# Gaurav14cs17/Bayer_Low_light_Image_Enhancement

Measured on AMD Instinct MI355X. Metric: megapixels/sec RawFormer-S 512x512 RAW->sRGB, higher is better.
Workload: dtype f32; 1 GPU; RawFormer-S(FLCA) dim=32, batch=8 of packed 4x512x512 synthetic Bayer per GPU; frames_per_gpu=8, variant=flca, weights=synthetic (seeded, random-init scale), parallelism=batch-sharded x1, device=AMD Radeon Graphics

## Files before the change

bayer_low_light_image_enhancement_amd/csrc/rf_gemm1x1.hip:

```cpp
#include <cstdio>
#include <cstdlib>
#include "rf_common.h"

namespace rf {

__device__ __forceinline__ const float* kset_base(const Conv1x1Args& a, int b, int s) {
    const int k = 4 * s;
    const bool first = k < a.C1;
    const float* src = first ? a.x1 : a.x2;
    const size_t off = (size_t)b * (size_t)(first ? a.x1_bstride : a.x2_bstride) + (size_t)(first ? k : k - a.C1) * (size_t)a.P;
    return src + off;
}

__device__ __forceinline__ float4 ldv(const float* __restrict__ base, unsigned off) {
    return *reinterpret_cast<const float4*>(base + off);
}

template <int NCO>
__device__ __forceinline__ void zero_acc(f32x4 (&acc)[NCO][4]) {
#pragma unroll
    for (int t = 0; t < NCO; ++t)
#pragma unroll
        for (int g = 0; g < 4; ++g) acc[t][g] = (f32x4){0.f, 0.f, 0.f, 0.f};
}

template <class BP>
__device__ __forceinline__ void b3_split_pair(float xa, float xb, BP& bp, int g, int hp) {
    unsigned a0, a1, a2, b0, b1, b2;
    b3_split(xa, a0, a1, a2);
    b3_split(xb, b0, b1, b2);
    bp[g][0][hp] = b3_pack(a0, b0);
    bp[g][1][hp] = b3_pack(a1, b1);
    bp[g][2][hp] = b3_pack(a2, b2);
}

template <int NCO, bool RES>
__device__ __forceinline__ void epilogue(const Conv1x1Args& a, f32x4 (&acc)[NCO][4], int tfirst, int ntiles,
                                         const float* __restrict__ bias_l, const float4* res,
                                         int b, int p0, int kq, bool live) {
    const int P = a.P;
    float* outb = a.out + (size_t)b * a.out_bstride;
    if (a.mode == 0) {
        const unsigned voff = (unsigned)(4 * kq) * (unsigned)P + (unsigned)p0;
#pragma unroll
        for (int t = 0; t < NCO; ++t) {
            if (t >= ntiles) break;
#pragma unroll
            for (int r = 0; r < 4; ++r) {
                const int cu = 16 * (tfirst + t) + r;
                const float bs = bias_l[16 * t + 4 * kq + r];
                float v[4] = {acc[t][0][r] + bs, acc[t][1][r] + bs, acc[t][2][r] + bs, acc[t][3][r] + bs};
                if constexpr (RES) {
                    const float4 rv = res[t * 4 + r];
                    v[0] += rv.x; v[1] += rv.y; v[2] += rv.z; v[3] += rv.w;
                }
                if (a.act == 1 || a.act == 3) {
                    const float slope = a.act == 1 ? 0.2f : 0.1f;
#pragma unroll
                    for (int g = 0; g < 4; ++g) v[g] = v[g] > 0.f ? v[g] : slope * v[g];
                } else if (a.act == 2) {
#pragma unroll
                    for (int g = 0; g < 4; ++g) v[g] = fmaxf(v[g], 0.f);
                } else if (a.act == 4) {
#pragma unroll
                    for (int g = 0; g < 4; ++g) v[g] = fminf(fmaxf(v[g], 0.f), 1e4f);
                }
                if (live && cu + 4 * kq < a.Cout)
                    *reinterpret_cast<float4*>(outb + (size_t)cu * P + voff) = make_float4(v[0], v[1], v[2], v[3]);
            }
        }
    } else {
        const int w = a.w, w2 = 2 * a.w;
        const int ya = p0 / w, xa = p0 - ya * w;
        const int yb = (p0 + 2) / w, xb = (p0 + 2) - yb * w;
#pragma unroll
        for (int t = 0; t < NCO; ++t) {
            if (t >= ntiles) break;
            const int co = 16 * (tfirst + t) + 4 * kq;
            const int o = co >> 2;
            const float bs = bias_l[4 * t + kq];
            float* op = outb + (size_t)o * 4 * P;
            if (live && co < a.Cout) {
#pragma unroll
                for (int i = 0; i < 2; ++i) {
                    *reinterpret_cast<float4*>(op + (size_t)(2 * ya + i) * w2 + 2 * xa) =
                        make_float4(acc[t][0][2 * i] + bs, acc[t][0][2 * i + 1] + bs, acc[t][1][2 * i] + bs, acc[t][1][2 * i + 1] + bs);
                    *reinterpret_cast<float4*>(op + (size_t)(2 * yb + i) * w2 + 2 * xb) =
                        make_float4(acc[t][2][2 * i] + bs, acc[t][2][2 * i + 1] + bs, acc[t][3][2 * i] + bs, acc[t][3][2 * i + 1] + bs);
                }
            }
        }
    }
}

__device__ __forceinline__ void stage_bias(const Conv1x1Args& a, float* bias_l, int tbeg, int tpad, int tid) {
    if (a.mode == 0) {
        for (int i = tid; i < tpad * 16; i += 256) {
            const int co = 16 * tbeg + i;
            bias_l[i] = (a.bias && co < a.Cout) ? a.bias[co] : 0.f;
        }
    } else {
        for (int i = tid; i < tpad * 4; i += 256) {
            const int o = 4 * tbeg + i;
            bias_l[i] = (a.bias && 4 * o < a.Cout) ? a.bias[o] : 0.f;
        }
    }
}

template <int KS, bool LN, int RT, bool DBUF>
__global__ void __launch_bounds__(256, (KS <= 8 ? 3 : 2)) conv1x1_res_kernel(Conv1x1Args a, int ntw, int ngroups) {
    constexpr int NCO = 2;
    constexpr bool RES = RT > 0;
    extern __shared__ __attribute__((aligned(16))) float lds[];
    const int tid = threadIdx.x;
    const int lane = tid & 63, wave = tid >> 6;
    const int j = lane & 15, kq = lane >> 4;
    const int grp = blockIdx.x % ngroups;
    const int wg = blockIdx.x / ngroups, nwg = gridDim.x / ngroups;
    const int b = blockIdx.y;
    const int P = a.P;
    const int K = a.C1 + a.C2;
    const int NS = K >> 2;
    const int NT = (a.Cout + 15) >> 4;
    const int tbeg = grp * ntw;
    const int tcnt = (NT - tbeg < ntw) ? NT - tbeg : ntw;
    const int tpad = (tcnt + NCO - 1) / NCO * NCO;
    const int ntiles = (P + 255) >> 8;
    float* lds_w = lds;
    float* bias_l = lds + KS * tpad * 64;
    float* gam_l = bias_l + tpad * 16;
    float* bet_l = gam_l + 4 * KS;

    auto load_tile = [&](int tile, float4 (&dst)[KS]) {
        const int p0 = (tile * 4 + wave) * 64 + 4 * j;
        const unsigned voff = (unsigned)kq * (unsigned)P + (unsigned)(p0 < P ? p0 : 0);
#pragma unroll
        for (int s = 0; s < KS; ++s) dst[s] = ldv(kset_base(a, b, s < NS ? s : NS - 1), voff);
    };

    float4 xr[KS], xn[DBUF ? KS : 1];
    int tile = wg;
    load_tile(tile < ntiles ? tile : 0, xr);
    {
        const float* wp = a.wp + (size_t)b * a.wp_bstride;
        const int n4 = KS * tpad * 16;
        for (int idx = tid; idx < n4; idx += 256) {
            const int l4 = idx & 15;
            const int t = (idx >> 4) % tpad;
            const int s = (idx >> 4) / tpad;
            float4 v = make_float4(0.f, 0.f, 0.f, 0.f);
            if (t < tcnt && s < NS) v = *reinterpret_cast<const float4*>(wp + ((size_t)s * NT + tbeg + t) * 64 + l4 * 4);
            *reinterpret_cast<float4*>(lds_w + ((size_t)s * tpad + t) * 64 + l4 * 4) = v;
        }
        stage_bias(a, bias_l, tbeg, tpad, tid);
        if constexpr (LN) {
            for (int i = tid; i < 4 * KS; i += 256) {
                gam_l[i] = i < K ? a.ln_w[i] : 0.f;
                bet_l[i] = (a.ln_b && i < K) ? a.ln_b[i] : 0.f;
            }
        }
    }
    __syncthreads();

    for (; tile < ntiles; tile += nwg) {
        const int p0 = (tile * 4 + wave) * 64 + 4 * j;
        const bool live = p0 < P;
        const int tnext = tile + nwg;
        if constexpr (DBUF) {
            load_tile(tnext < ntiles ? tnext : tile, xn);
        }
        float4 res[RES ? RT * 4 : 1];
        if constexpr (RES) {
            const float* resb = a.res + (size_t)b * a.res_bstride;
            const unsigned voff = (unsigned)(4 * kq) * (unsigned)P + (unsigned)(live ? p0 : 0);
#pragma unroll
            for (int t = 0; t < RT; ++t)
#pragma unroll
                for (int r = 0; r < 4; ++r)
                    res[t * 4 + r] = ldv(resb + (size_t)(16 * (tbeg + (t < tcnt ? t : tcnt - 1)) + r) * P, voff);
        }
        if constexpr (LN) {
            float sum[4] = {0.f, 0.f, 0.f, 0.f};
#pragma unroll
            for (int s = 0; s < KS; ++s)
                if (s < NS) { sum[0] += xr[s].x; sum[1] += xr[s].y; sum[2] += xr[s].z; sum[3] += xr[s].w; }
            const float invK = 1.0f / (float)K;
            float mu[4], var[4] = {0.f, 0.f, 0.f, 0.f};
#pragma unroll
            for (int g = 0; g < 4; ++g) {
                sum[g] += __shfl_xor(sum[g], 16);
                sum[g] += __shfl_xor(sum[g], 32);
                mu[g] = sum[g] * invK;
            }
#pragma unroll
            for (int s = 0; s < KS; ++s) {
                if (s < NS) {
                    const float d0 = xr[s].x - mu[0], d1 = xr[s].y - mu[1], d2 = xr[s].z - mu[2], d3 = xr[s].w - mu[3];
                    var[0] = fmaf(d0, d0, var[0]); var[1] = fmaf(d1, d1, var[1]);
                    var[2] = fmaf(d2, d2, var[2]); var[3] = fmaf(d3, d3, var[3]);
                }
            }
            float rstd[4], sh[4];
#pragma unroll
            for (int g = 0; g < 4; ++g) {
                var[g] += __shfl_xor(var[g], 16);
                var[g] += __shfl_xor(var[g], 32);
                rstd[g] = 1.0f / sqrtf(var[g] * invK + a.ln_eps);
                sh[g] = a.ln_b ? mu[g] : 0.f;
            }
#pragma unroll
            for (int s = 0; s < KS; ++s) {
                const float gk = gam_l[4 * s + kq], bk = bet_l[4 * s + kq];
                xr[s].x = fmaf((xr[s].x - sh[0]) * rstd[0], gk, bk);
                xr[s].y = fmaf((xr[s].y - sh[1]) * rstd[1], gk, bk);
                xr[s].z = fmaf((xr[s].z - sh[2]) * rstd[2], gk, bk);
                xr[s].w = fmaf((xr[s].w - sh[3]) * rstd[3], gk, bk);
            }
        }
        auto do_group = [&](int tg, const float4* resp) {
            f32x4 acc[NCO][4];
            zero_acc(acc);
            const float* wl = lds_w + (size_t)tg * 64 + lane;
#pragma unroll
            for (int s = 0; s < KS; ++s) {
                const float xb[4] = {xr[s].x, xr[s].y, xr[s].z, xr[s].w};
#pragma unroll
                for (int t = 0; t < NCO; ++t) {
                    const float av = wl[((size_t)s * tpad + t) * 64];
#pragma unroll
                    for (int g = 0; g < 4; ++g)
                        acc[t][g] = __builtin_amdgcn_mfma_f32_16x16x4f32(av, xb[g], acc[t][g], 0, 0, 0);
                }
            }
            epilogue<NCO, RES>(a, acc, tbeg + tg, tcnt - tg, bias_l + (a.mode == 0 ? 16 : 4) * tg, resp, b, p0, kq, live);
        };
        if constexpr (RES) {
            do_group(0, &res[0]);
            if constexpr (RT > NCO) {
                if (tpad > NCO) do_group(NCO, &res[NCO * 4]);
            }
        } else {
#pragma unroll 1
            for (int tg = 0; tg < tpad; tg += NCO) do_group(tg, res);
        }
        if constexpr (DBUF) {
#pragma unroll
            for (int s = 0; s < KS; ++s) xr[s] = xn[s];
        } else {
            if (tnext < ntiles) load_tile(tnext, xr);
        }
    }
}

static constexpr int kStreamLnMaxK = 1024;

template <int NCO, int KCH, bool LN>
__global__ void __launch_bounds__(256, 2) conv1x1_stream_kernel(Conv1x1Args a, int ngroups) {
    __shared__ __attribute__((aligned(16))) float lds_w[2][KCH * NCO * 64];
    __shared__ float bias_l[NCO * 16];
    __shared__ float gam_l[LN ? kStreamLnMaxK : 4], bet_l[LN ? kStreamLnMaxK : 4];
    constexpr int WPT = KCH * NCO * 16 / 256;
    static_assert(KCH * NCO * 16 % 256 == 0, "weight chunk must split evenly over the workgroup");
    const int tid = threadIdx.x;
    const int lane = tid & 63, wave = tid >> 6;
    const int j = lane & 15, kq = lane >> 4;
    const int grp = blockIdx.x % ngroups;
    const int tile = blockIdx.x / ngroups;
    const int b = blockIdx.y;
    const int P = a.P;
    const int K = a.C1 + a.C2;
    const int NS = K >> 2;
    const int NT = (a.Cout + 15) >> 4;
    const int t0 = grp * NCO;
    const int tcnt = (NT - t0 < NCO) ? NT - t0 : NCO;
    const int nch = (NS + KCH - 1) / KCH;
    const int p0 = (tile * 4 + wave) * 64 + 4 * j;
    const bool live = p0 < P;
    const unsigned voff = (unsigned)kq * (unsigned)P + (unsigned)(live ? p0 : 0);
    const float* wp = a.wp + (size_t)b * a.wp_bstride;
    stage_bias(a, bias_l, t0, NCO, tid);
    if constexpr (LN) {
        for (int i = tid; i < 4 * nch * KCH; i += 256) {
            gam_l[i] = i < K ? a.ln_w[i] : 0.f;
            bet_l[i] = (a.ln_b && i < K) ? a.ln_b[i] : 0.f;
        }
    }

    f32x4 acc[NCO][4];
    zero_acc(acc);
    if (a.res && a.mode == 0) {
        const float* resb = a.res + (size_t)b * a.res_bstride;
        const unsigned vo = (unsigned)(live ? p0 : 0);
#pragma unroll
        for (int t = 0; t < NCO; ++t)
#pragma unroll
            for (int r = 0; r < 4; ++r) {
                const int co = 16 * (t0 + t) + 4 * kq + r;
                const bool ok = live && t < tcnt && co < a.Cout;
                const float4 rv = ldv(resb + (size_t)(ok ? co : 0) * P, vo);
                acc[t][0][r] = ok ? rv.x : 0.f; acc[t][1][r] = ok ? rv.y : 0.f;
                acc[t][2][r] = ok ? rv.z : 0.f; acc[t][3][r] = ok ? rv.w : 0.f;
            }
    }

    float lnA[4] = {1.f, 1.f, 1.f, 1.f}, lnB[4] = {0.f, 0.f, 0.f, 0.f};
    if constexpr (LN) {
        const float4 s4 = ldv(kset_base(a, b, 0), (unsigned)(live ? p0 : 0));
        const float sh[4] = {s4.x, s4.y, s4.z, s4.w};
        float s1[4] = {0.f, 0.f, 0.f, 0.f}, s2[4] = {0.f, 0.f, 0.f, 0.f};
#pragma unroll 16
        for (int s = 0; s < NS; ++s) {
            const float4 t = ldv(kset_base(a, b, s), voff);
            const float d[4] = {t.x - sh[0], t.y - sh[1], t.z - sh[2], t.w - sh[3]};
#pragma unroll
            for (int g = 0; g < 4; ++g) { s1[g] += d[g]; s2[g] = fmaf(d[g], d[g], s2[g]); }
        }
        const float invK = 1.0f / (float)K;
#pragma unroll
        for (int g = 0; g < 4; ++g) {
            s1[g] += __shfl_xor(s1[g], 16); s1[g] += __shfl_xor(s1[g], 32);
            s2[g] += __shfl_xor(s2[g], 16); s2[g] += __shfl_xor(s2[g], 32);
            const float md = s1[g] * invK;
            const float var = fmaxf(fmaf(-md, md, s2[g] * invK), 0.f);
            const float rstd = 1.0f / sqrtf(var + a.ln_eps);
            lnA[g] = rstd;
            lnB[g] = a.ln_b ? -(sh[g] + md) * rstd : 0.f;
        }
    }

    float4 xa[KCH], xb_[KCH], wr[WPT];
    auto load_x_chunk = [&](int c, float4 (&dst)[KCH]) {
#pragma unroll
        for (int i = 0; i < KCH; ++i) {
            const int s = c * KCH + i;
            dst[i] = ldv(kset_base(a, b, s < NS ? s : NS - 1), voff);
        }
    };
    auto load_w_chunk = [&](int c) {
#pragma unroll
        for (int i = 0; i < WPT; ++i) {
            const int idx = tid + 256 * i;
            const int l4 = idx & 15, t = (idx >> 4) % NCO, s = c * KCH + (idx >> 4) / NCO;
            const bool ok = s < NS && t < tcnt;
            const float4 v = *reinterpret_cast<const float4*>(wp + ((size_t)(ok ? s : 0) * NT + t0 + (ok ? t : 0)) * 64 + l4 * 4);
            wr[i] = ok ? v : make_float4(0.f, 0.f, 0.f, 0.f);
        }
    };
    auto store_w_chunk = [&](int buf) {
#pragma unroll
        for (int i = 0; i < WPT; ++i) *reinterpret_cast<float4*>(&lds_w[buf][(tid + 256 * i) * 4]) = wr[i];
    };
    auto chunk = [&](int c, float4 (&xc)[KCH], float4 (&xn)[KCH]) {
        if (c + 1 < nch) {
            load_x_chunk(c + 1, xn);
            load_w_chunk(c + 1);
        }
        const float* wl = &lds_w[c & 1][lane];
#pragma unroll
        for (int i = 0; i < KCH; ++i) {
            float xv[4] = {xc[i].x, xc[i].y, xc[i].z, xc[i].w};
            if constexpr (LN) {
                const int k = 4 * (c * KCH + i) + kq;
                const float gk = gam_l[k], bk = bet_l[k];
#pragma unroll
                for (int g = 0; g < 4; ++g) xv[g] = fmaf(fmaf(xv[g], lnA[g], lnB[g]), gk, bk);
            }
#pragma unroll
            for (int t = 0; t < NCO; ++t) {
                const float av = wl[(i * NCO + t) * 64];
#pragma unroll
                for (int g = 0; g < 4; ++g)
                    acc[t][g] = __builtin_amdgcn_mfma_f32_16x16x4f32(av, xv[g], acc[t][g], 0, 0, 0);
            }
        }
        if (c + 1 < nch) store_w_chunk((c + 1) & 1);
        __syncthreads();
    };

    load_x_chunk(0, xa);
    load_w_chunk(0);
    store_w_chunk(0);
    __syncthreads();
    for (int c = 0; c < nch; c += 2) {
        chunk(c, xa, xb_);
        if (c + 1 < nch) chunk(c + 1, xb_, xa);
    }
    epilogue<NCO, false>(a, acc, t0, tcnt, bias_l, nullptr, b, p0, kq, live);
}


__device__ __forceinline__ void b3_load_x_block(float4 (&xr)[8], const float* xb1, const float* xb2, const float* xb3, int C1, int C2, int C3,
                                                int c, int kq, unsigned P, unsigned pl) {
    const int cb = 32 * c;
    const bool first = cb < C1, third = cb >= C1 + C2;
    const float* src = first ? xb1 : third ? xb3 : xb2;
    const int cloc = first ? cb : third ? cb - C1 - C2 : cb - C1, cmax = (first ? C1 : third ? C3 : C2) - 1;
#pragma unroll
    for (int i = 0; i < 8; ++i) {
        int ch = cloc + 8 * kq + i;
        ch = ch < cmax ? ch : cmax;
        xr[i] = ldv(src, (unsigned)ch * P + pl);
    }
}

template <int NCO, bool LN, bool PAIR = false>
__global__ void __launch_bounds__(PAIR ? 512 : 256, 2) conv1x1_b3_kernel(Conv1x1Args a, int ngroups) {
    static_assert(!(PAIR && LN), "the paired form has no LayerNorm prologue");
    constexpr int NH = PAIR ? 2 : 1;
    __shared__ __attribute__((aligned(16))) u32x4 lds_w[NH * 2][NCO * 3 * 64];
    __shared__ float bias_l[NH * NCO * 16];
    __shared__ float gam_l[LN ? kStreamLnMaxK : 4], bet_l[LN ? kStreamLnMaxK : 4];
    constexpr int WPT = (NCO * 3 * 64 + 255) / 256;
    const int tid = PAIR ? threadIdx.x & 255 : threadIdx.x;
    const int half = PAIR ? threadIdx.x >> 8 : 0;
    const int lane = tid & 63, wave = tid >> 6;
    const int j = lane & 15, kq = lane >> 4;
    unsigned unit = 0, gp = 0, utiles = 1;
    if constexpr (PAIR) {
        utiles = (unsigned)(a.P + 255) >> 8;
        if (!conv1x1_group_map(blockIdx.x, (unsigned)a.B * utiles, (unsigned)(ngroups + 1) >> 1, &unit, &gp)) return;
    }
    const int grp = PAIR ? 2 * (int)gp + half : blockIdx.x % ngroups;
    const int tile = PAIR ? unit % utiles : blockIdx.x / ngroups;
    const int b = PAIR ? unit / utiles : blockIdx.y;
    const int P = a.P;
    const int K = a.C1 + a.C2 + a.C3;
    const int NB = (K + 31) >> 5;
    const int NT = (a.Cout + 15) >> 4;
    const bool idle = PAIR && grp >= ngroups;
    const int t0 = idle ? 0 : grp * NCO;
    const int tcnt = idle ? 0 : (NT - t0 < NCO) ? NT - t0 : NCO;
    const int p0 = (tile * 4 + wave) * 64 + 4 * j;
    const bool live = p0 < P;
    const unsigned pl = (unsigned)(live ? p0 : 0);
    const u32x4* wp3 = reinterpret_cast<const u32x4*>(reinterpret_cast<const float*>(a.wp3) + (size_t)b * a.wp3_bstride);
    stage_bias(a, bias_l + half * NCO * 16, t0, NCO, tid);
    if constexpr (LN) {
        for (int i = tid; i < 32 * NB; i += 256) {
            gam_l[i] = i < K ? a.ln_w[i] : 0.f;
            bet_l[i] = (a.ln_b && i < K) ? a.ln_b[i] : 0.f;
        }
    }

    f32x4 acc[NCO][4];
#pragma unroll
    for (int t = 0; t < NCO; ++t)
#pragma unroll
        for (int g = 0; g < 4; ++g) acc[t][g] = (f32x4){0.f, 0.f, 0.f, 0.f};
    if (a.res && a.mode == 0) {
        const float* resb = a.res + (size_t)b * a.res_bstride;
#pragma unroll
        for (int t = 0; t < NCO; ++t)
#pragma unroll
            for (int r = 0; r < 4; ++r) {
                const int co = 16 * (t0 + t) + 4 * kq + r;
                const bool ok = live && t < tcnt && co < a.Cout;
                const float4 rv = ldv(resb + (size_t)(ok ? co : 0) * P, pl);
                acc[t][0][r] = ok ? rv.x : 0.f; acc[t][1][r] = ok ? rv.y : 0.f;
                acc[t][2][r] = ok ? rv.z : 0.f; acc[t][3][r] = ok ? rv.w : 0.f;
            }
    }

    float lnA[4] = {1.f, 1.f, 1.f, 1.f}, lnB[4] = {0.f, 0.f, 0.f, 0.f};
    if constexpr (LN) {
        const unsigned voff = (unsigned)kq * (unsigned)P + pl;
        const float4 s4 = ldv(kset_base(a, b, 0), pl);
        const float sh[4] = {s4.x, s4.y, s4.z, s4.w};
        float s1[4] = {0.f, 0.f, 0.f, 0.f}, s2[4] = {0.f, 0.f, 0.f, 0.f};
#pragma unroll 16
        for (int s = 0; s < (K >> 2); ++s) {
            const float4 t = ldv(kset_base(a, b, s), voff);
            const float d[4] = {t.x - sh[0], t.y - sh[1], t.z - sh[2], t.w - sh[3]};
#pragma unroll
            for (int g = 0; g < 4; ++g) { s1[g] += d[g]; s2[g] = fmaf(d[g], d[g], s2[g]); }
        }
        const float invK = 1.0f / (float)K;
#pragma unroll
        for (int g = 0; g < 4; ++g) {
            s1[g] += __shfl_xor(s1[g], 16); s1[g] += __shfl_xor(s1[g], 32);
            s2[g] += __shfl_xor(s2[g], 16); s2[g] += __shfl_xor(s2[g], 32);
            const float md = s1[g] * invK;
            const float var = fmaxf(fmaf(-md, md, s2[g] * invK), 0.f);
            const float rstd = 1.0f / sqrtf(var + a.ln_eps);
            lnA[g] = rstd;
            lnB[g] = a.ln_b ? -(sh[g] + md) * rstd : 0.f;
        }
    }

    float4 xr[8];
    u32x4 wr[WPT];
    const float* const xb1 = a.x1 + (size_t)b * (size_t)a.x1_bstride;
    const float* const xb2 = a.x2 + (size_t)b * (size_t)a.x2_bstride;
    const float* const xb3 = a.x3 + (size_t)b * (size_t)a.x3_bstride;
    auto load_x_block = [&](int c) { b3_load_x_block(xr, xb1, xb2, xb3, a.C1, a.C2, a.C3, c, kq, (unsigned)P, pl); };
    auto load_w_block = [&](int c) {
#pragma unroll
        for (int i = 0; i < WPT; ++i) {
            const int idx = tid + 256 * i;
            const int t = idx / 192, rem = idx - t * 192;
            const bool ok = idx < NCO * 192 && t < tcnt;
            const u32x4 v = wp3[((size_t)c * NT + t0 + (ok ? t : 0)) * 192 + (ok ? rem : 0)];
            wr[i] = ok ? v : (u32x4){0u, 0u, 0u, 0u};
        }
    };
    auto store_w_block = [&](int buf) {
#pragma unroll
        for (int i = 0; i < WPT; ++i)
            if (tid + 256 * i < NCO * 192) lds_w[2 * half + buf][tid + 256 * i] = wr[i];
    };

    load_x_block(0);
    load_w_block(0);
    store_w_block(0);
    __syncthreads();
    for (int c = 0; c < NB; ++c) {
        u32x4 bp[4][3];
#pragma unroll
        for (int hp = 0; hp < 4; ++hp) {
            float xa[4] = {xr[2 * hp].x, xr[2 * hp].y, xr[2 * hp].z, xr[2 * hp].w};
            float xb[4] = {xr[2 * hp + 1].x, xr[2 * hp + 1].y, xr[2 * hp + 1].z, xr[2 * hp + 1].w};
            if constexpr (LN) {
                const int k = 32 * c + 8 * kq + 2 * hp;
                const float ga = gam_l[k], ba = bet_l[k], gb = gam_l[k + 1], bb = bet_l[k + 1];
#pragma unroll
                for (int g = 0; g < 4; ++g) {
                    xa[g] = fmaf(fmaf(xa[g], lnA[g], lnB[g]), ga, ba);
                    xb[g] = fmaf(fmaf(xb[g], lnA[g], lnB[g]), gb, bb);
                }
            }
#pragma unroll
            for (int g = 0; g < 4; ++g) b3_split_pair(xa[g], xb[g], bp, g, hp);
        }
        if (c + 1 < NB) {
            load_x_block(c + 1);
            load_w_block(c + 1);
        }
        const u32x4* wl = &lds_w[2 * half + (c & 1)][lane];
#pragma unroll
        for (int t = 0; t < NCO; ++t) {
            const u32x4 ap[3] = {wl[(t * 3 + 0) * 64], wl[(t * 3 + 1) * 64], wl[(t * 3 + 2) * 64]};
            b3_mfma4(ap, bp, acc[t]);
        }
        if (c + 1 < NB) store_w_block((c + 1) & 1);
        __syncthreads();
    }
    epilogue<NCO, false>(a, acc, t0, tcnt, bias_l + half * NCO * 16, nullptr, b, p0, kq, live);
}

template <int KB, int NCO>
__global__ void __launch_bounds__(256, KB <= 4 ? 2 : 1) conv1x1_b3_ln_kernel(Conv1x1Args a, int tpw) {
    __shared__ __attribute__((aligned(16))) u32x4 Bl[KB * 768];
    __shared__ __attribute__((aligned(16))) float red[2 * 4 * 64];
    __shared__ float bias_l[1024];
    constexpr int KPW = KB >= 4 ? KB / 4 : 1;
    constexpr int CPT = KB >= 4 ? 8 : 4;
    constexpr int K = 32 * KB;
    const int tid = threadIdx.x, lane = tid & 63, wave = tid >> 6;
    const int j = lane & 15, kq = lane >> 4;
    const int b = blockIdx.y, P = a.P;
    const int NT = a.Cout >> 4;
    const int ntile = (P + 63) >> 6;
    const float* xb = a.x1 + (size_t)b * a.x1_bstride;
    const u32x4* wp3 = reinterpret_cast<const u32x4*>(reinterpret_cast<const float*>(a.wp3) + (size_t)b * a.wp3_bstride) + lane;
    for (int i = tid; i < a.Cout; i += 256) bias_l[i] = a.bias ? a.bias[i] : 0.f;

    const int kb0 = KB >= 4 ? wave * KPW : wave >> 1;
    const int cbase = KB >= 4 ? 8 * kq : 8 * kq + 4 * (wave & 1);
    float4 xr[KPW][CPT];
    auto load_x = [&](int tile) {
        const int q0 = tile * 64 + 4 * j;
        const unsigned ql = (unsigned)(q0 < P ? q0 : 0);
#pragma unroll
        for (int i = 0; i < KPW; ++i)
#pragma unroll
            for (int c = 0; c < CPT; ++c) xr[i][c] = ldv(xb, (unsigned)(32 * (kb0 + i) + cbase + c) * (unsigned)P + ql);
    };
    constexpr bool PREF = KB != 4;
    if (PREF) load_x(blockIdx.x);
    for (int tile = blockIdx.x; tile < ntile; tile += gridDim.x) {
    if (!PREF) load_x(tile);
    const int p0 = tile * 64 + 4 * j;
    const bool live = p0 < P;
    float mean[4], rstd[4];
    {
        float s[4] = {0.f, 0.f, 0.f, 0.f};
#pragma unroll
        for (int i = 0; i < KPW; ++i)
#pragma unroll
            for (int c = 0; c < CPT; ++c) { s[0] += xr[i][c].x; s[1] += xr[i][c].y; s[2] += xr[i][c].z; s[3] += xr[i][c].w; }
#pragma unroll
        for (int g = 0; g < 4; ++g) { s[g] += __shfl_xor(s[g], 16); s[g] += __shfl_xor(s[g], 32); }
        if (kq == 0) *reinterpret_cast<float4*>(red + wave * 64 + 4 * j) = make_float4(s[0], s[1], s[2], s[3]);
        __syncthreads();
        const float4 r0 = *reinterpret_cast<const float4*>(red + 4 * j), r1 = *reinterpret_cast<const float4*>(red + 64 + 4 * j);
        const float4 r2 = *reinterpret_cast<const float4*>(red + 128 + 4 * j), r3 = *reinterpret_cast<const float4*>(red + 192 + 4 * j);
        mean[0] = (((r0.x + r1.x) + r2.x) + r3.x) * (1.0f / K); mean[1] = (((r0.y + r1.y) + r2.y) + r3.y) * (1.0f / K);
        mean[2] = (((r0.z + r1.z) + r2.z) + r3.z) * (1.0f / K); mean[3] = (((r0.w + r1.w) + r2.w) + r3.w) * (1.0f / K);
        float v[4] = {0.f, 0.f, 0.f, 0.f};
#pragma unroll
        for (int i = 0; i < KPW; ++i)
#pragma unroll
            for (int c = 0; c < CPT; ++c) {
                const float d0 = xr[i][c].x - mean[0], d1 = xr[i][c].y - mean[1], d2 = xr[i][c].z - mean[2], d3 = xr[i][c].w - mean[3];
                v[0] = fmaf(d0, d0, v[0]); v[1] = fmaf(d1, d1, v[1]); v[2] = fmaf(d2, d2, v[2]); v[3] = fmaf(d3, d3, v[3]);
            }
#pragma unroll
        for (int g = 0; g < 4; ++g) { v[g] += __shfl_xor(v[g], 16); v[g] += __shfl_xor(v[g], 32); }
        if (kq == 0) *reinterpret_cast<float4*>(red + 256 + wave * 64 + 4 * j) = make_float4(v[0], v[1], v[2], v[3]);
        __syncthreads();
        const float4 q0 = *reinterpret_cast<const float4*>(red + 256 + 4 * j), q1 = *reinterpret_cast<const float4*>(red + 320 + 4 * j);
        const float4 q2 = *reinterpret_cast<const float4*>(red + 384 + 4 * j), q3 = *reinterpret_cast<const float4*>(red + 448 + 4 * j);
        rstd[0] = 1.0f / sqrtf((((q0.x + q1.x) + q2.x) + q3.x) * (1.0f / K) + a.ln_eps);
        rstd[1] = 1.0f / sqrtf((((q0.y + q1.y) + q2.y) + q3.y) * (1.0f / K) + a.ln_eps);
        rstd[2] = 1.0f / sqrtf((((q0.z + q1.z) + q2.z) + q3.z) * (1.0f / K) + a.ln_eps);
        rstd[3] = 1.0f / sqrtf((((q0.w + q1.w) + q2.w) + q3.w) * (1.0f / K) + a.ln_eps);
    }
#pragma unroll
    for (int i = 0; i < KPW; ++i) {
        const int kb = kb0 + i;
        unsigned bpd[4][3][CPT / 2];
#pragma unroll
        for (int hp = 0; hp < CPT / 2; ++hp) {
            const int k = 32 * kb + cbase + 2 * hp;
            const float ga = a.ln_w[k], gb = a.ln_w[k + 1];
            const float ba = a.ln_b ? a.ln_b[k] : 0.f, bb = a.ln_b ? a.ln_b[k + 1] : 0.f;
            const float xa[4] = {xr[i][2 * hp].x, xr[i][2 * hp].y, xr[i][2 * hp].z, xr[i][2 * hp].w};
            const float xc[4] = {xr[i][2 * hp + 1].x, xr[i][2 * hp + 1].y, xr[i][2 * hp + 1].z, xr[i][2 * hp + 1].w};
#pragma unroll
            for (int g = 0; g < 4; ++g) {
                const float mu = a.ln_b ? mean[g] : 0.f;
                b3_split_pair(fmaf((xa[g] - mu) * rstd[g], ga, ba), fmaf((xc[g] - mu) * rstd[g], gb, bb), bpd, g, hp);
            }
        }
#pragma unroll
        for (int g = 0; g < 4; ++g)
#pragma unroll
            for (int pc = 0; pc < 3; ++pc) {
                u32x4* dst = &Bl[((kb * 4 + g) * 3 + pc) * 64 + lane];
                if constexpr (CPT == 8) *dst = (u32x4){bpd[g][pc][0], bpd[g][pc][1], bpd[g][pc][2], bpd[g][pc][3]};
                else reinterpret_cast<uint2*>(dst)[wave & 1] = make_uint2(bpd[g][pc][0], bpd[g][pc][1]);
            }
    }
    __syncthreads();
    if (PREF && tile + (int)gridDim.x < ntile) load_x(tile + gridDim.x);

    for (int chunk = 0; chunk * NCO < tpw; ++chunk) {
        const int t0 = ((int)blockIdx.z * 4 + wave) * tpw + chunk * NCO;
        f32x4 acc[NCO][4];
#pragma unroll
        for (int t = 0; t < NCO; ++t)
#pragma unroll
            for (int g = 0; g < 4; ++g) acc[t][g] = (f32x4){0.f, 0.f, 0.f, 0.f};
        constexpr int STEPS = KB * NCO, RING = KB > 4 ? 12 : (STEPS < 5 ? STEPS : 5);
        u32x4 A[RING][3];
        auto load_a = [&](int slot, int step) {
            const int kb = step / NCO, t = step - kb * NCO;
#pragma unroll
            for (int pc = 0; pc < 3; ++pc) A[slot][pc] = wp3[((size_t)kb * NT + t0 + t) * 192 + pc * 64];
        };
#pragma unroll
        for (int i = 0; i < RING - 1; ++i) load_a(i, i);
        u32x4 bp[2][4][3];
        auto load_b = [&](int buf, int kb, int first, int last) {
#pragma unroll
            for (int i = first; i < last; ++i) bp[buf][i / 3][i % 3] = Bl[(kb * 12 + i) * 64 + lane];
        };
        load_b(0, 0, 0, 12);
#pragma unroll
        for (int step = 0; step < STEPS; ++step) {
            const int kb = step / NCO, t = step % NCO;
            if (step + RING - 1 < STEPS) load_a((step + RING - 1) % RING, step + RING - 1);
            if (kb + 1 < KB) load_b((kb + 1) & 1, kb + 1, 12 * t / NCO, 12 * (t + 1) / NCO);
            b3_mfma4(A[step % RING], bp[kb & 1], acc[t]);
            __builtin_amdgcn_sched_barrier(0);
        }
        epilogue<NCO, false>(a, acc, t0, NCO, bias_l + 16 * t0, nullptr, b, p0, kq, live);
    }
    }
}

__global__ void __launch_bounds__(256) conv1x1_scalar_kernel(Conv1x1Args a) {
    const int P = a.P, K = a.C1 + a.C2, NT = (a.Cout + 15) >> 4;
    const int b = blockIdx.y;
    const float* wp = a.wp + (size_t)b * a.wp_bstride;
    for (int p = blockIdx.x * 256 + threadIdx.x; p < P; p += gridDim.x * 256) {
        auto xat = [&](int k) {
            return (k < a.C1) ? a.x1[(size_t)b * a.x1_bstride + (size_t)k * P + p]
                              : a.x2[(size_t)b * a.x2_bstride + (size_t)(k - a.C1) * P + p];
        };
        float mu = 0.f, rstd = 1.f;
        if (a.ln_w) {
            for (int k = 0; k < K; ++k) mu += xat(k);
            mu /= (float)K;
            float var = 0.f;
            for (int k = 0; k < K; ++k) { const float d = xat(k) - mu; var = fmaf(d, d, var); }
            rstd = 1.0f / sqrtf(var / (float)K + a.ln_eps);
            if (!a.ln_b) mu = 0.f;
        }
        for (int co = 0; co < a.Cout; ++co) {
            float s = 0.f;
            for (int k = 0; k < K; ++k) {
                float xv = xat(k);
                if (a.ln_w) xv = fmaf((xv - mu) * rstd, a.ln_w[k], a.ln_b ? a.ln_b[k] : 0.f);
                s = fmaf(wp[((size_t)(k >> 2) * NT + (co >> 4)) * 64 + (co & 15) + 16 * (k & 3)], xv, s);
            }
            if (a.mode == 0) {
                s += a.bias ? a.bias[co] : 0.f;
                if (a.res) s += a.res[(size_t)b * a.res_bstride + (size_t)co * P + p];
                if (a.act == 1) s = s > 0.f ? s : 0.2f * s;
                else if (a.act == 2) s = fmaxf(s, 0.f);
                else if (a.act == 3) s = s > 0.f ? s : 0.1f * s;
                else if (a.act == 4) s = fminf(fmaxf(s, 0.f), 1e4f);
                a.out[(size_t)b * a.out_bstride + (size_t)co * P + p] = s;
            } else {
                const int o = co >> 2, y = p / a.w, x = p - y * a.w;
                s += a.bias ? a.bias[o] : 0.f;
                a.out[(size_t)b * a.out_bstride + (size_t)o * 4 * P + (size_t)(2 * y + ((co >> 1) & 1)) * (2 * a.w) + 2 * x + (co & 1)] = s;
            }
        }
    }
}

enum { kScalar, kRes, kStream, kB3, kB3Ln };
struct Conv1x1Inst {
    const char* key;
    int family, targ[4];
    unsigned block;
    void (*launch)(const Conv1x1Args&, const Conv1x1Plan&, hipStream_t);
};
#define RF_GRID dim3(p.grid[0], p.grid[1], p.grid[2]), p.block, p.lds, st
#define RF_INST(FAMILY, BLOCK, KERNEL, KARGS, ...)                                      \
    {#KERNEL "<" #__VA_ARGS__ ">", FAMILY, {__VA_ARGS__}, BLOCK,                        \
     [](const Conv1x1Args& a, const Conv1x1Plan& p, hipStream_t st) { KERNEL<__VA_ARGS__><<<RF_GRID>>> KARGS; }}
#define RF_RES(...) RF_INST(kRes, 256, conv1x1_res_kernel, (a, p.karg[0], p.karg[1]), __VA_ARGS__)
#define RF_RES6(KS, DBUF4)              \
    RF_RES(KS, true, 4, DBUF4), RF_RES(KS, false, 4, DBUF4), RF_RES(KS, true, 2, true), RF_RES(KS, false, 2, true), RF_RES(KS, true, 0, true), RF_RES(KS, false, 0, true)
#define RF_STREAM(...) RF_INST(kStream, 256, conv1x1_stream_kernel, (a, p.karg[0]), __VA_ARGS__)
#define RF_B3(BLOCK, ...) RF_INST(kB3, BLOCK, conv1x1_b3_kernel, (a, p.karg[0]), __VA_ARGS__)
#define RF_B3LN(...) RF_INST(kB3Ln, 256, conv1x1_b3_ln_kernel, (a, p.karg[0]), __VA_ARGS__)
static const Conv1x1Inst kInst[] = {
    {"conv1x1_scalar_kernel", kScalar, {}, 256, [](const Conv1x1Args& a, const Conv1x1Plan& p, hipStream_t st) { conv1x1_scalar_kernel<<<RF_GRID>>>(a); }},
    RF_B3LN(2, 3), RF_B3LN(2, 2), RF_B3LN(4, 3), RF_B3LN(4, 2), RF_B3LN(8, 4), RF_B3LN(8, 3), RF_B3LN(8, 2),
    RF_B3(512, 6, false, true), RF_B3(512, 4, false, true), RF_B3(256, 6, false), RF_B3(256, 2, false), RF_B3(256, 4, true), RF_B3(256, 4, false),
    RF_RES6(4, true), RF_RES6(8, true), RF_RES6(12, false), RF_RES6(16, false),
    RF_RES(24, false, 0, false), RF_RES(32, false, 0, false),
    RF_STREAM(8, 4, true), RF_STREAM(8, 4, false), RF_STREAM(4, 8, true), RF_STREAM(4, 8, false),
};
#undef RF_GRID

static int find_inst(int family, int t0, int t1, int t2, Conv1x1Plan* p) {
    const int want[3] = {t0, t1, t2};
    for (const Conv1x1Inst& r : kInst) {
        bool ok = r.family == family;
        for (int k = 0; k < 3; ++k) ok = ok && (want[k] < 0 || want[k] == r.targ[k]);
        if (ok) { p->inst = (int)(&r - kInst); p->key = r.key; p->block = r.block; return RF_OK; }
    }
    RF_CHECK_ARG(false, "conv1x1: no kernel instantiation for family %d <%d, %d, %d>", family, t0, t1, t2);
}

static bool b3_ln_supported(const Conv1x1Args& a, int* nco) {
    const int K = a.C1 + a.C2;
    if (!(a.ln_w && a.wp3 && a.C2 == 0 && (K == 64 || K == 128 || K == 256) && a.mode == 0 && !a.res && a.Cout % 64 == 0 && a.Cout <= 1024 &&
          aligned16(a.wp3) && a.wp3_bstride % 4 == 0))
        return false;
    const int tpw = a.Cout / 64;
    *nco = (K == 256 && tpw % 4 == 0) ? 4 : tpw % 3 == 0 ? 3 : tpw % 2 == 0 ? 2 : 0;
    return *nco != 0;
}

static bool b3_supported(const Conv1x1Args& a) {
    const int K = a.C1 + a.C2 + a.C3;
    return K >= 128 && a.C1 % 8 == 0 && a.C2 % 8 == 0 && a.C3 % 8 == 0 && (a.C2 + a.C3 == 0 || a.C1 % 32 == 0) &&
           (a.C3 == 0 || a.C2 % 32 == 0) && (!a.ln_w || (K <= kStreamLnMaxK && a.C3 == 0)) && aligned16(a.wp3) && (a.wp3_bstride % 4 == 0);
}

int plan_conv1x1(const Conv1x1Args& a, Conv1x1Plan* p) {
    bool b3_ok = a.wp3 != nullptr;
    int force_pair = -1;
#ifdef RF_DIAG
    if (getenv("RF_NO_B3")) b3_ok = false;
    if (const char* e = getenv("RF_B3_PAIR")) force_pair = e[0] != '0';
#endif
    RF_CHECK_ARG(a.B > 0 && a.P > 0 && a.C1 > 0 && a.C2 >= 0 && a.Cout > 0, "conv1x1: bad sizes B=%d P=%d C1=%d C2=%d Cout=%d",
                 a.B, a.P, a.C1, a.C2, a.Cout);
    RF_CHECK_ARG(a.C1 % 4 == 0 && a.C2 % 4 == 0, "conv1x1: input channel counts (%d, %d) must be multiples of 4", a.C1, a.C2);
    RF_CHECK_ARG(a.C2 == 0 || a.x2 != nullptr, "conv1x1: second source missing");
    RF_CHECK_ARG(a.C3 >= 0 && a.C3 % 4 == 0 && (a.C3 == 0 || (a.x3 != nullptr && a.C2 > 0)), "conv1x1: bad third source (C3 = %d)", a.C3);
    RF_CHECK_ARG(a.mode == 0 || (a.Cout % 4 == 0 && a.w > 0 && a.P % a.w == 0 && !a.res), "conv1x1: bad ConvTranspose geometry");
    RF_CHECK_ARG(a.B <= 65535 && (double)a.P * 4.0 * 16.0 < 4.0e9, "conv1x1: batch %d / plane %d too large", a.B, a.P);
    const int K = a.C1 + a.C2 + a.C3;
    const int NS = K / 4, NT = cdiv(a.Cout, 16);
    const int ptiles = cdiv(a.P, 256);
    const long units = (long)ptiles * a.B;
    bool vec = (a.P % 4 == 0) && aligned16(a.x1) && aligned16(a.out) && (a.x1_bstride % 4 == 0) && (a.out_bstride % 4 == 0);
    if (a.x2) vec = vec && aligned16(a.x2) && (a.x2_bstride % 4 == 0);
    if (a.C3) vec = vec && aligned16(a.x3) && (a.x3_bstride % 4 == 0);
    if (a.res) vec = vec && aligned16(a.res) && (a.res_bstride % 4 == 0);
    if (a.mode == 1) vec = vec && (a.w % 2 == 0);
    const bool ln = a.ln_w != nullptr;
    const double px = (double)a.B * a.P;
    *p = Conv1x1Plan{};
    p->flops = 2.0 * K * a.Cout * px;
    p->bytes = 4.0 * px * (K + a.Cout + (a.res ? a.Cout : 0));
    p->grid[1] = (unsigned)a.B; p->grid[2] = 1;
    int nco_ln = 0;
    const bool ln_once = b3_ln_supported(a, &nco_ln);
    p->ln_single_pass = !ln || a.C1 + a.C2 <= 64 || ln_once;
    const bool use_b3 = b3_ok && b3_supported(a);
    RF_CHECK_ARG(a.C3 == 0 || (use_b3 && vec && !a.ln_w && !(a.res && a.Cout % 16 != 0)), "conv1x1: three sources need the bf16x3 kernel (K = %d, P = %d)", K, a.P);
    if (!vec || (a.res && a.Cout % 16 != 0) || (ln && K > kStreamLnMaxK)) {
        p->grid[0] = (unsigned)(cdiv(a.P, 256) < 4096 ? cdiv(a.P, 256) : 4096);
        return find_inst(kScalar, -1, -1, -1, p);
    }
    if (b3_ok && ln_once) {
        const int kb = K / 32;
        int tpw = a.Cout / 64;
        const int slots = (kb <= 4 ? 2 : 1) * 256;
        int gx = slots / a.B;
        gx = gx < 1 ? 1 : gx;
        gx = gx < cdiv(a.P, 64) ? gx : cdiv(a.P, 64);
        int zs = 1;
        if ((long)gx * a.B < 128)
            for (int z = tpw / nco_ln; z > 1; --z)
                if ((tpw / nco_ln) % z == 0 && (long)gx * a.B * z <= 512) { zs = z; break; }
        p->grid[0] = (unsigned)gx; p->grid[2] = (unsigned)zs;
        p->karg[0] = tpw / zs;
        return find_inst(kB3Ln, kb, nco_ln, -1, p);
    }
    if (use_b3) {
        int nco = (!ln && (NT % 6 == 0 || (NT % 4 != 0 && NT > 8))) ? 6 : 4;
        const bool pair = !ln && cdiv(NT, nco) > 1 && (force_pair >= 0 ? force_pair != 0 : units * cdiv(cdiv(NT, nco), 2) >= 256);
        if (!pair && !ln && nco == 4 && NT % 2 == 0 && units * cdiv(NT, 4) < 256) nco = 2;
        const int ngroups = cdiv(NT, nco);
        const long pair_ids = (units + 7) / 8 * 8 * cdiv(ngroups, 2);
        RF_CHECK_ARG(!pair || pair_ids < (1L << 31), "conv1x1: %ld pixel tiles x %d output groups is too large a grid", units, ngroups);
        p->karg[0] = ngroups;
        if (pair) { p->grid[0] = conv1x1_group_grid((unsigned)units, (unsigned)cdiv(ngroups, 2)); p->grid[1] = 1; }
        else p->grid[0] = (unsigned)(ptiles * ngroups);
        return find_inst(kB3, nco, ln, pair, p);
    }
    if (NS <= 16 || (NS <= 32 && !ln && !a.res)) {
        const int ks = NS <= 4 ? 4 : NS <= 8 ? 8 : NS <= 12 ? 12 : NS <= 16 ? 16 : NS <= 24 ? 24 : 32;
        int cap = (240 / ks) & ~1;
        if (a.res && cap > 4) cap = 4;
        if (a.res && (ks <= 8 || ln) && cap > 2) cap = 2;
        const int ntw = NT < cap ? NT : cap;
        const int ngroups = cdiv(NT, ntw);
        const int tpad = cdiv(ntw, 2) * 2;
        p->lds = ((size_t)ks * tpad * 64 + tpad * 16 + 8 * ks) * sizeof(float);
        const int slots = 256 * (ks <= 8 ? 3 : 2);
        int wgs = cdiv(slots, a.B * ngroups);
        if (wgs > ptiles) wgs = ptiles;
        p->grid[0] = (unsigned)(wgs * ngroups);
        p->karg[0] = ntw; p->karg[1] = ngroups;
        return find_inst(kRes, ks, ln, a.res ? (ntw > 2 ? 4 : 2) : 0, p);
    }
    int nco = (NT % 8 == 0 || NT > 12) ? 8 : 4;
    if (nco == 8) {
        const long cost8 = ((units * cdiv(NT, 8) + 511) / 512) * 8, cost4 = ((units * cdiv(NT, 4) + 511) / 512) * 4;
        if (cost4 < cost8) nco = 4;
    }
    p->karg[0] = cdiv(NT, nco);
    p->grid[0] = (unsigned)(ptiles * p->karg[0]);
    return find_inst(kStream, nco, -1, ln, p);
}

bool conv1x1_ln_single_pass(const Conv1x1Args& a) {
    Conv1x1Plan p;
    return plan_conv1x1(a, &p) != RF_OK || p.ln_single_pass;
}

int launch_conv1x1(const Conv1x1Args& a, hipStream_t st) {
    Conv1x1Plan p;
    RF_TRY(plan_conv1x1(a, &p));
    {
        ProfScope prof(st, p.key, p.flops, p.bytes);
        kInst[p.inst].launch(a, p, st);
    }
    return check_launch("conv1x1");
}

}
```

Baseline: 1107 MP/s.

## Restructure LN+1x1 conv kernel with cross-tile weight/activation prefetch and resident weights

Moves the LayerNorm-fused 1x1 GEMM body into a templated device function. A RESIDENT variant keeps all weight fragments in registers across tiles when KB==2 and one chunk per wave. Otherwise the next tile's activations and the next chunk's weights are prefetched inside the MFMA loop, so global-load latency overlaps compute across tiles and chunks. It also caches LN gamma/beta in registers, inlines a simplified epilogue with precomputed store offsets, and uses readfirstlane for the wave index. The cost is higher register pressure, which could lower occupancy or cause spills, and the epilogue now stores unconditionally using clamped offsets.

```diff
diff --git a/bayer_low_light_image_enhancement_amd/csrc/rf_gemm1x1.hip b/bayer_low_light_image_enhancement_amd/csrc/rf_gemm1x1.hip
--- a/bayer_low_light_image_enhancement_amd/csrc/rf_gemm1x1.hip
+++ b/bayer_low_light_image_enhancement_amd/csrc/rf_gemm1x1.hip
@@ -1,5 +1,6 @@
 #include <cstdio>
 #include <cstdlib>
+#include <type_traits>
 #include "rf_common.h"
 
 namespace rf {
@@ -547,40 +548,68 @@
     epilogue<NCO, false>(a, acc, t0, tcnt, bias_l + half * NCO * 16, nullptr, b, p0, kq, live);
 }
 
-template <int KB, int NCO>
-__global__ void __launch_bounds__(256, KB <= 4 ? 2 : 1) conv1x1_b3_ln_kernel(Conv1x1Args a, int tpw) {
-    __shared__ __attribute__((aligned(16))) u32x4 Bl[KB * 768];
-    __shared__ __attribute__((aligned(16))) float red[2 * 4 * 64];
-    __shared__ float bias_l[1024];
+template <int KB, int NCO, bool RESIDENT>
+__device__ __forceinline__ void b3_ln_tiles(const Conv1x1Args& a, const int tpw, u32x4* __restrict__ Bl, float* __restrict__ red,
+                                            const float* __restrict__ bias_l) {
     constexpr int KPW = KB >= 4 ? KB / 4 : 1;
     constexpr int CPT = KB >= 4 ? 8 : 4;
     constexpr int K = 32 * KB;
-    const int tid = threadIdx.x, lane = tid & 63, wave = tid >> 6;
+    constexpr int STEPS = KB * NCO, RING = RESIDENT ? STEPS : KB > 4 ? 12 : (STEPS < 5 ? STEPS : 5);
+    constexpr int AHEAD = RESIDENT ? STEPS : RING - 1;
+    constexpr int XSTEP = (KB == 4 && NCO == 3) ? STEPS - NCO : STEPS - RING;
+    const int tid = threadIdx.x, lane = tid & 63, wave = __builtin_amdgcn_readfirstlane(tid >> 6);
     const int j = lane & 15, kq = lane >> 4;
     const int b = blockIdx.y, P = a.P;
     const int NT = a.Cout >> 4;
     const int ntile = (P + 63) >> 6;
+    const int tw0 = ((int)blockIdx.z * 4 + wave) * tpw;
     const float* xb = a.x1 + (size_t)b * a.x1_bstride;
-    const u32x4* wp3 = reinterpret_cast<const u32x4*>(reinterpret_cast<const float*>(a.wp3) + (size_t)b * a.wp3_bstride) + lane;
-    for (int i = tid; i < a.Cout; i += 256) bias_l[i] = a.bias ? a.bias[i] : 0.f;
+    float* outb = a.out + (size_t)b * a.out_bstride;
+    const char* wp3 = reinterpret_cast<const char*>(reinterpret_cast<const float*>(a.wp3) + (size_t)b * a.wp3_bstride);
+    const unsigned aoff = 16u * (unsigned)lane;
 
     const int kb0 = KB >= 4 ? wave * KPW : wave >> 1;
-    const int cbase = KB >= 4 ? 8 * kq : 8 * kq + 4 * (wave & 1);
+    const int cwave = KB >= 4 ? 0 : 4 * (wave & 1);
+    const int cbase = 8 * kq + cwave;
     float4 xr[KPW][CPT];
-    auto load_x = [&](int tile) {
+    auto load_x = [&](int tile, bool exists) {
         const int q0 = tile * 64 + 4 * j;
-        const unsigned ql = (unsigned)(q0 < P ? q0 : 0);
+        size_t xoff = exists ? (size_t)(8 * kq) * (size_t)P + (size_t)(q0 < P ? q0 : tile * 64) : (size_t)0;
+        asm volatile("" : "+v"(xoff));
 #pragma unroll
         for (int i = 0; i < KPW; ++i)
 #pragma unroll
-            for (int c = 0; c < CPT; ++c) xr[i][c] = ldv(xb, (unsigned)(32 * (kb0 + i) + cbase + c) * (unsigned)P + ql);
+            for (int c = 0; c < CPT; ++c) xr[i][c] = *reinterpret_cast<const float4*>(xb + (size_t)(32 * (kb0 + i) + cwave + c) * (size_t)P + xoff);
     };
-    constexpr bool PREF = KB != 4;
-    if (PREF) load_x(blockIdx.x);
+    u32x4 A[RING][3];
+    auto load_a = [&](int slot, int step, int t0) {
+        const int kb = step / NCO, t = step - kb * NCO;
+#pragma unroll
+        for (int pc = 0; pc < 3; ++pc)
+            A[slot][pc] = *reinterpret_cast<const u32x4*>(wp3 + (((size_t)kb * NT + t0 + t) * 192 + pc * 64) * 16 + aoff);
+    };
+    load_x(blockIdx.x, true);
+#pragma unroll
+    for (int i = 0; i < AHEAD; ++i) load_a(i, i, tw0);
+    constexpr bool LNREG = KB != 4;
+    float gam[LNREG ? KPW : 1][CPT], bet[LNREG ? KPW : 1][CPT];
+    if constexpr (LNREG) {
+#pragma unroll
+        for (int i = 0; i < KPW; ++i)
+#pragma unroll
+            for (int c = 0; c < CPT; ++c) {
+                const int k = 32 * (kb0 + i) + cbase + c;
+                gam[i][c] = a.ln_w[k];
+                bet[i][c] = a.ln_b ? a.ln_b[k] : 0.f;
+            }
+    }
+    __builtin_amdgcn_s_waitcnt(0x0F70);
+
     for (int tile = blockIdx.x; tile < ntile; tile += gridDim.x) {
-    if (!PREF) load_x(tile);
-    const int p0 = tile * 64 + 4 * j;
-    const bool live = p0 < P;
+    const int tnext = tile + (int)gridDim.x;
+    const bool more = tnext < ntile;
+    const int q0 = tile * 64 + 4 * j;
+    const int p0 = q0 < P ? q0 : tile * 64;
     float mean[4], rstd[4];
     {
         float s[4] = {0.f, 0.f, 0.f, 0.f};
@@ -622,8 +651,8 @@
 #pragma unroll
         for (int hp = 0; hp < CPT / 2; ++hp) {
             const int k = 32 * kb + cbase + 2 * hp;
-            const float ga = a.ln_w[k], gb = a.ln_w[k + 1];
-            const float ba = a.ln_b ? a.ln_b[k] : 0.f, bb = a.ln_b ? a.ln_b[k + 1] : 0.f;
+            const float ga = LNREG ? gam[LNREG ? i : 0][2 * hp] : a.ln_w[k], gb = LNREG ? gam[LNREG ? i : 0][2 * hp + 1] : a.ln_w[k + 1];
+            const float ba = LNREG ? bet[LNREG ? i : 0][2 * hp] : a.ln_b ? a.ln_b[k] : 0.f, bb = LNREG ? bet[LNREG ? i : 0][2 * hp + 1] : a.ln_b ? a.ln_b[k + 1] : 0.f;
             const float xa[4] = {xr[i][2 * hp].x, xr[i][2 * hp].y, xr[i][2 * hp].z, xr[i][2 * hp].w};
             const float xc[4] = {xr[i][2 * hp + 1].x, xr[i][2 * hp + 1].y, xr[i][2 * hp + 1].z, xr[i][2 * hp + 1].w};
 #pragma unroll
@@ -642,24 +671,17 @@
             }
     }
     __syncthreads();
-    if (PREF && tile + (int)gridDim.x < ntile) load_x(tile + gridDim.x);
-
-    for (int chunk = 0; chunk * NCO < tpw; ++chunk) {
-        const int t0 = ((int)blockIdx.z * 4 + wave) * tpw + chunk * NCO;
+    if constexpr (RESIDENT) load_x(tnext, more);
+    unsigned soff = 4u * ((unsigned)(4 * kq) * (unsigned)P + (unsigned)p0);
+    asm volatile("" : "+v"(soff));
+
+    auto run_chunk = [&](const int t0, auto last_chunk) {
+        constexpr bool LAST = decltype(last_chunk)::value;
         f32x4 acc[NCO][4];
 #pragma unroll
         for (int t = 0; t < NCO; ++t)
 #pragma unroll
             for (int g = 0; g < 4; ++g) acc[t][g] = (f32x4){0.f, 0.f, 0.f, 0.f};
-        constexpr int STEPS = KB * NCO, RING = KB > 4 ? 12 : (STEPS < 5 ? STEPS : 5);
-        u32x4 A[RING][3];
-        auto load_a = [&](int slot, int step) {
-            const int kb = step / NCO, t = step - kb * NCO;
-#pragma unroll
-            for (int pc = 0; pc < 3; ++pc) A[slot][pc] = wp3[((size_t)kb * NT + t0 + t) * 192 + pc * 64];
-        };
-#pragma unroll
-        for (int i = 0; i < RING - 1; ++i) load_a(i, i);
         u32x4 bp[2][4][3];
         auto load_b = [&](int buf, int kb, int first, int last) {
 #pragma unroll
@@ -669,14 +691,58 @@
 #pragma unroll
         for (int step = 0; step < STEPS; ++step) {
             const int kb = step / NCO, t = step % NCO;
-            if (step + RING - 1 < STEPS) load_a((step + RING - 1) % RING, step + RING - 1);
+            if constexpr (!RESIDENT) {
+                if (step + RING - 1 < STEPS) load_a((step + RING - 1) % RING, step + RING - 1, t0);
+                if (LAST && step == XSTEP) {
+                    __builtin_amdgcn_sched_barrier(0);
+                    load_x(tnext, more);
+                }
+            }
             if (kb + 1 < KB) load_b((kb + 1) & 1, kb + 1, 12 * t / NCO, 12 * (t + 1) / NCO);
             b3_mfma4(A[step % RING], bp[kb & 1], acc[t]);
             __builtin_amdgcn_sched_barrier(0);
         }
-        epilogue<NCO, false>(a, acc, t0, NCO, bias_l + 16 * t0, nullptr, b, p0, kq, live);
-    }
-    }
+        if constexpr (!RESIDENT) {
+#pragma unroll
+            for (int i = 0; i < RING - 1; ++i) load_a(i, i, LAST ? tw0 : t0 + NCO);
+            __builtin_amdgcn_sched_barrier(0);
+        }
+#pragma unroll
+        for (int t = 0; t < NCO; ++t)
+#pragma unroll
+            for (int r = 0; r < 4; ++r) {
+                const float bs = bias_l[16 * (t0 + t) + 4 * kq + r];
+                float v[4] = {acc[t][0][r] + bs, acc[t][1][r] + bs, acc[t][2][r] + bs, acc[t][3][r] + bs};
+                if (a.act == 1 || a.act == 3) {
+                    const float slope = a.act == 1 ? 0.2f : 0.1f;
+#pragma unroll
+                    for (int g = 0; g < 4; ++g) v[g] = v[g] > 0.f ? v[g] : slope * v[g];
+                } else if (a.act == 2) {
+#pragma unroll
+                    for (int g = 0; g < 4; ++g) v[g] = fmaxf(v[g], 0.f);
+                } else if (a.act == 4) {
+#pragma unroll
+                    for (int g = 0; g < 4; ++g) v[g] = fminf(fmaxf(v[g], 0.f), 1e4f);
+                }
+                *reinterpret_cast<float4*>(reinterpret_cast<char*>(outb + (size_t)(16 * (t0 + t) + r) * (size_t)P) + soff) = make_float4(v[0], v[1], v[2], v[3]);
+            }
+    };
+    if constexpr (!RESIDENT)
+        for (int t0 = tw0; t0 + NCO < tw0 + tpw; t0 += NCO) run_chunk(t0, std::false_type{});
+    run_chunk(tw0 + tpw - NCO, std::true_type{});
+    }
+}
+
+template <int KB, int NCO>
+__global__ void __launch_bounds__(256, KB <= 4 ? 2 : 1) conv1x1_b3_ln_kernel(Conv1x1Args a, int tpw) {
+    __shared__ __attribute__((aligned(16))) u32x4 Bl[KB * 768];
+    __shared__ __attribute__((aligned(16))) float red[2 * 4 * 64];
+    __shared__ float bias_l[1024];
+    for (int i = threadIdx.x; i < a.Cout; i += 256) bias_l[i] = a.bias ? a.bias[i] : 0.f;
+    if constexpr (KB == 2) {
+        if (tpw == NCO) return b3_ln_tiles<KB, NCO, true>(a, tpw, Bl, red, bias_l);
+    }
+    b3_ln_tiles<KB, NCO, false>(a, tpw, Bl, red, bias_l);
 }
 
 __global__ void __launch_bounds__(256) conv1x1_scalar_kernel(Conv1x1Args a) {
```

New measurement: 1130 MP/s, median of 6. 1.02x the previous value.
